# sasg/cilium

Hardware: AMD Instinct MI355X
Metric: classified headers/sec (Mpps, whole node) at 100k-prefix ipcache + 16k-ID policy (higher is better)
Workload: dtype u32

## Files before the change

### cilium_amd/csrc/classify.hip

```cpp
#include <algorithm>
#include <cstdlib>
#include <mutex>
#include <set>
#include <tuple>
#include <vector>

#include "kern_common.hpp"
#ifndef CFC_EXP
#define CFC_EXP 0
#endif

namespace cfc {

namespace {

constexpr int LDS_MET_U64 = 18;
template <int MODE>
constexpr int met_n()
{
    return MODE == CFC_MODE_EGRESS ? 7 : MODE == CFC_MODE_XDP ? 0 : 4;
}
template <int MODE>
constexpr int acc_n()
{
// ... 684 lines not shown
                          out.notify, o4);
                if (CT) {
                    sto_nt(h[u].ct_k1, C.ct, o4);
                    if (EGR)
                        sto_nt(h[u].ct_k2, C.ct2, o4);
                }
                if (LB && out.pkt_saddr) {
                    sto_nt(h[u].psa, out.pkt_saddr, o4);
                    sto_nt(h[u].da, out.pkt_daddr, o4);
                    sto_nt(h[u].ppt, out.pkt_ports, o4);
                }
                if (MODE != CFC_MODE_XDP) {
#if CFC_EXP != 3
                    if (!kc_ctr) {
                        sto_nt(ctr_key(C, h[u].ctr0, len), C.ctr, o4);
                        if (EGR)
                            sto_nt(ctr_key(C, h[u].ctr1, len), C.ctr2, o4);
                    }
                    if (!KC)
                        sto_nt(h[u].idw, C.id, o4);
#endif
                }
            }
#if CFC_EXP != 3
            if (MODE != CFC_MODE_XDP) {
                if (kc_ctr) {
                    key_append(ctr_key(C, h[u].ctr0, len), h[u].valid, C.ctr, kn_ctr);
                    if (EGR)
                        key_append(ctr_key(C, h[u].ctr1, len), h[u].valid, C.ctr2, kn_ctr2);
                }
                if (KC)
                    key_append(h[u].idw, h[u].valid, C.id, kn_id);
            }
#endif
            if (WL && E.wbits) {
                bool pr;
                const bool w = wl_want<EGR>(h[u].ct_byte, h[u].ver, h[u].mt, h[u].ct_k1,
                                            EGR ? h[u].ct_k2 : NONE, pr);
                const uint64_t wb = __ballot(w && h[u].valid), pb = __ballot(pr && h[u].valid);
                const uint32_t w0 = base + u * BLOCK + (threadIdx.x & ~63u);
                if ((threadIdx.x & 63) == 0 && w0 < end) {
                    E.wbits[(start + w0) >> 6] = wb;
                    E.wprobe[(start + w0) >> 6] = pb;
                }
            }
            if (MODE != CFC_MODE_XDP && E.nat_idx)
                list_append(E.nat_idx, E.nat_cnt, h[u].nat && h[u].valid, (uint32_t)start + i);
            if (MODE != CFC_MODE_XDP && h[u].valid && h[u].id_ovf && h[u].need_pol)
                id_count(C, id_dir, h[u].ident, h[u].drop1, len);
            if (LBE && h[u].valid && h[u].ver == DROP_NO_SERVICE) {
                unsigned long long *m = reinterpret_cast<unsigned long long *>(
                    C.g_met + (uint64_t)(-DROP_NO_SERVICE * METRIC_DIRS + METRIC_EGRESS) * 2);
                atomicAdd(m, 1ull);
                atomicAdd(m + 1, (unsigned long long)len);
            }
#if CFC_EXP != 5
            acc.add(h[u].valid ? h[u].met0 : NONE, len);
#endif
            if (EGR) {
                acc.add(h[u].valid ? h[u].met1 : NONE, len);
                acc.add(h[u].valid && h[u].ev2 ? met_n<MODE>() + h[u].ev2 - 1 : NONE, len);
            }
        }
        if (++iter == 65536 / (2 * U)) {
            acc.flush(s_met);
            iter = 0;
        }
    }
    acc.flush(s_met);
    if (CFC_KEYS_COMPACT && MODE != CFC_MODE_XDP && (threadIdx.x & 63) == 0) {
        const uint32_t wave = key_wave();
        const uint64_t to_counts =
            (uint64_t)(gridDim.x - blockIdx.x) * per_block -
            (uint64_t)wave * key_regions_grid(gridDim.x, per_block).cap +
            (uint64_t)blockIdx.x * KEY_WAVES + wave;
        if (kc_ctr) {
            C.ctr[to_counts] = kn_ctr;
            if (EGR)
                C.ctr2[to_counts] = kn_ctr2;
        }
        if (KC)
            C.id[to_counts] = kn_id;
    }
    __syncthreads();
    acc_publish<MODE>(s_met, C, E.seclabel);
}

}

namespace {

struct HistJob {
    const uint32_t *keys;
    uint64_t poff;
    uint32_t lo, cnt;
    uint32_t kind;
    uint32_t packed;
    uint32_t compact, cap;
    const uint32_t *counts;
    uint64_t n, per_block;
};
constexpr int HIST_JOBS_MAX = 12;
struct HistJobs {
    HistJob j[HIST_JOBS_MAX];
};
constexpr uint64_t SLICE_MAX = 1ull << 31;

__device__ __forceinline__ unsigned long long *hist_dst(const HistJob &jb, uint32_t key,
                                                        uint64_t *g_ctr, uint64_t *g_id,
                                                        uint32_t id_dir)
{
    return reinterpret_cast<unsigned long long *>(
        jb.kind == 0 ? g_ctr + 2ull * key : g_id + id_index(id_dir, key >> 1, key & 1));
}

struct HistLds {
    uint32_t *ek, *ec, *ew;
    uint32_t *s;
};
__device__ __forceinline__ HistLds hist_lds()
{
    uint32_t *b = reinterpret_cast<uint32_t *>(cfc_smem);
    return HistLds{b, b + HIST_ESC_SLOTS, b + 2 * HIST_ESC_SLOTS, b + 3 * HIST_ESC_SLOTS};
}

struct HistAdd {
    uint32_t r, len, old;
};
__device__ __forceinline__ HistAdd hist_add(uint32_t *s, const HistJob &jb, uint32_t w,
                                            uint32_t m)
{
    HistAdd a;
    uint32_t k;
    if (jb.packed) {
        k = w & 0xFFFF;
        a.len = w >> 16;
    } else {
        k = w;
        a.len = m >> 16;
    }
    a.r = k - jb.lo;
    a.old = a.r < jb.cnt && w != KEY_NONE ? atomicAdd(&s[a.r], HistSlot::inc(a.len)) : 0u;
    return a;
}
__device__ __forceinline__ bool hist_spills(const HistAdd &a)
{
    uint32_t carry, wrap;
    HistSlot::spill(a.old, a.len, carry, wrap);
    return (carry | wrap) != 0;
}
__device__ __forceinline__ void hist_escape(const HistLds &L, const HistJob &jb,
                                            const HistAdd &a, uint64_t *g_ctr, uint64_t *g_id,
                                            uint32_t id_dir)
{
    uint32_t carry, wrap;
    HistSlot::spill(a.old, a.len, carry, wrap);
    if (!(carry | wrap))
        return;
    uint32_t h = fmix32(a.r) & (HIST_ESC_SLOTS - 1);
    for (int p = 0; p < 8; p++) {
        uint32_t cur = L.ek[h];
        if (cur == NONE) {
            cur = atomicCAS(&L.ek[h], NONE, a.r);
            if (cur == NONE)
                cur = a.r;
        }
        if (cur == a.r) {
            if (carry)
                atomicAdd(&L.ec[h], carry);
            if (wrap)
                atomicAdd(&L.ew[h], wrap);
            return;
        }
        h = (h + 1) & (HIST_ESC_SLOTS - 1);
    }
    unsigned long long *d = hist_dst(jb, jb.lo + a.r, g_ctr, g_id, id_dir);
    atomicAdd(d, (unsigned long long)HistSlot::esc_packets(carry, wrap));
    if (carry)
        atomicAdd(d + 1, (unsigned long long)HistSlot::esc_bytes(carry));
}

__device__ __forceinline__ void hist_compact(const HistLds &L, const HistJob &jb,
                                             uint64_t start, uint64_t stop, uint64_t *g_ctr,
                                             uint64_t *g_id, uint32_t id_dir)
{
    if (start >= stop)
        return;
    const uint32_t wave = __builtin_amdgcn_readfirstlane(threadIdx.x >> 6);
    const uint32_t lane4 = 4 * (threadIdx.x & 63);
    const uint32_t r1 = (uint32_t)((stop + jb.cap - 1) / jb.cap);
    uint32_t r = (uint32_t)(start / jb.cap) + wave;
    uint32_t cnt = r < r1 ? jb.counts[r] : 0u;
    while (r < r1) {
        const uint32_t rn = r + KEY_WAVES;
        const uint32_t cnt_n = rn < r1 ? jb.counts[rn] : 0u;
        const uint64_t rb = (uint64_t)r * jb.cap;
        const uint64_t lo = max(rb, start), hi = min(rb + min(cnt, jb.cap), stop);
        if (lo < hi) {
            const uint32_t len = (uint32_t)(hi - lo), last = (len - 1) & ~3u;
            const uint32_t *k = jb.keys + lo;
            uint4 w0 = ld_nt4(k + min(lane4, last));
            uint4 w1 = ld_nt4(k + min(lane4 + 256, last));
            for (uint32_t o = lane4, b = 0; b < len; b += 256, o += 256) {
                const uint4 w2 = ld_nt4(k + min(o + 512, last));
                const HistAdd a0 = hist_add(L.s, jb, o < len ? w0.x : KEY_NONE, 0u);
                const HistAdd a1 = hist_add(L.s, jb, o + 1 < len ? w0.y : KEY_NONE, 0u);
                const HistAdd a2 = hist_add(L.s, jb, o + 2 < len ? w0.z : KEY_NONE, 0u);
                const HistAdd a3 = hist_add(L.s, jb, o + 3 < len ? w0.w : KEY_NONE, 0u);
                if (hist_spills(a0) | hist_spills(a1) | hist_spills(a2) | hist_spills(a3)) {
                    hist_escape(L, jb, a0, g_ctr, g_id, id_dir);
                    hist_escape(L, jb, a1, g_ctr, g_id, id_dir);
                    hist_escape(L, jb, a2, g_ctr, g_id, id_dir);
                    hist_escape(L, jb, a3, g_ctr, g_id, id_dir);
                }
                w0 = w1;
                w1 = w2;
            }
        }
        r = rn;
        cnt = cnt_n;
    }
}

__global__ __launch_bounds__(BLOCK) void k_hist(HistJobs J, const uint32_t *meta,
                                                uint32_t *partial, uint64_t *g_ctr,
                                                uint64_t *g_id, uint32_t id_dir)
{
    const HistJob jb = J.j[blockIdx.y];
    const HistLds L = hist_lds();
    uint32_t *s = L.s;
    for (uint32_t j = threadIdx.x; j < HIST_ESC_SLOTS; j += BLOCK) {
        L.ek[j] = NONE;
        L.ec[j] = 0;
        L.ew[j] = 0;
    }
    for (uint32_t j = threadIdx.x; j < jb.cnt; j += BLOCK)
        s[j] = 0;
    __syncthreads();
    const uint64_t start = (uint64_t)blockIdx.x * jb.per_block;
    const uint64_t stop = max(start, min(jb.n, start + jb.per_block));
    if (jb.compact)
        hist_compact(L, jb, start, stop, g_ctr, g_id, id_dir);
    const uint64_t end = jb.compact ? start : stop;
    const uint64_t end4 = start + ((end - start) & ~3ull);
    const bool meta16 = (reinterpret_cast<uintptr_t>(meta) & 15) == 0;
    auto load = [&](uint64_t i, uint4 &w, uint4 &m) {
        w = make_uint4(KEY_NONE, KEY_NONE, KEY_NONE, KEY_NONE);
        m = make_uint4(0, 0, 0, 0);
        if (i >= end4)
            return;
        w = ld_nt4(jb.keys + i);
        if (!jb.packed) {
            if (meta16) {
                m = ld_nt4(meta + i);
            } else {
                m.x = meta[i];
                m.y = meta[i + 1];
                m.z = meta[i + 2];
                m.w = meta[i + 3];
            }
        }
    };
    const uint64_t i0 = start + 4 * threadIdx.x;
    uint4 w0, m0, w1, m1;
    load(i0, w0, m0);
    load(i0 + 4 * BLOCK, w1, m1);
    for (uint64_t i = i0; i < end4; i += 4 * BLOCK) {
        uint4 w2, m2;
        load(i + 8 * BLOCK, w2, m2);
        const HistAdd a0 = hist_add(s, jb, w0.x, m0.x);
        const HistAdd a1 = hist_add(s, jb, w0.y, m0.y);
        const HistAdd a2 = hist_add(s, jb, w0.z, m0.z);
        const HistAdd a3 = hist_add(s, jb, w0.w, m0.w);
        if (hist_spills(a0) | hist_spills(a1) | hist_spills(a2) | hist_spills(a3)) {
            hist_escape(L, jb, a0, g_ctr, g_id, id_dir);
            hist_escape(L, jb, a1, g_ctr, g_id, id_dir);
            hist_escape(L, jb, a2, g_ctr, g_id, id_dir);
            hist_escape(L, jb, a3, g_ctr, g_id, id_dir);
        }
        w0 = w1; m0 = m1;
        w1 = w2; m1 = m2;
    }
    for (uint64_t i = end4 + threadIdx.x; i < end; i += BLOCK) {
        const HistAdd a = hist_add(s, jb, jb.keys[i], jb.packed ? 0u : meta[i]);
        if (hist_spills(a))
            hist_escape(L, jb, a, g_ctr, g_id, id_dir);
    }
    __syncthreads();
    uint32_t *dst = partial + jb.poff + (uint64_t)blockIdx.x * jb.cnt;
    for (uint32_t j = threadIdx.x; j < jb.cnt; j += BLOCK)
        st_nt(s[j], dst + j);
    for (uint32_t j = threadIdx.x; j < HIST_ESC_SLOTS; j += BLOCK) {
        const uint32_t r = L.ek[j];
        if (r == NONE)
            continue;
        const uint32_t carries = L.ec[j], wraps = L.ew[j];
        unsigned long long *d = hist_dst(jb, jb.lo + r, g_ctr, g_id, id_dir);
        atomicAdd(d, (unsigned long long)HistSlot::esc_packets(carries, wraps));
        if (carries)
            atomicAdd(d + 1, (unsigned long long)HistSlot::esc_bytes(carries));
    }
}

constexpr uint32_t REDUCE_ROWS = 32;
__global__ __launch_bounds__(256) void k_hist_reduce(HistJobs J, const uint32_t *partial,
                                                     uint32_t nblk, uint64_t *g_ctr,
                                                     uint64_t *g_id, uint32_t id_dir)
{
    const HistJob jb = J.j[blockIdx.y];
    const uint32_t j = blockIdx.x * 256 + threadIdx.x;
    if (j >= jb.cnt)
        return;
    uint64_t pk = 0, by = 0;
    const uint32_t *p = partial + jb.poff + j;
    const uint32_t b0 = blockIdx.z * REDUCE_ROWS, b1 = min(nblk, b0 + REDUCE_ROWS);
    for (uint32_t b = b0; b < b1; b++) {
        const uint32_t v = ld_nt(p + (uint64_t)b * jb.cnt);
        pk += HistSlot::packets(v);
        by += HistSlot::bytes(v);
    }
    if (!(pk | by))
        return;
    unsigned long long *dst = hist_dst(jb, jb.lo + j, g_ctr, g_id, id_dir);
    if (pk)
        atomicAdd(dst, (unsigned long long)pk);
    if (by)
        atomicAdd(dst + 1, (unsigned long long)by);
}

constexpr uint32_t CT_LDS_SLOTS = 8192;
constexpr uint32_t CT_LDS_BYTES = CT_LDS_SLOTS * 12;
__global__ __launch_bounds__(BLOCK) void k_ct_count(const uint32_t *ct_idx,
                                                    const uint32_t *ct_idx2,
                                                    const uint32_t *meta,
                                                    uint64_t n,
                                                    CtState *st)
{
    uint32_t *keys = reinterpret_cast<uint32_t *>(cfc_smem);
    unsigned long long *vals =
        reinterpret_cast<unsigned long long *>(keys + CT_LDS_SLOTS);
    for (uint32_t j = threadIdx.x; j < CT_LDS_SLOTS; j += BLOCK) {
        keys[j] = NONE;
        vals[j] = 0;
    }
    __syncthreads();
    const uint32_t *idx = blockIdx.y ? ct_idx2 : ct_idx;
    const uint64_t start = (uint64_t)blockIdx.x * COUNT_PER_BLOCK;
    const uint64_t end = min(n, start + COUNT_PER_BLOCK);
    for (uint64_t i = start + threadIdx.x; i < end; i += BLOCK) {
        const uint32_t k = ld_nt(idx + i);
        if (k >= CK_MISS)
            continue;
        const uint32_t len = ld_nt(meta + i) >> 16;
        uint32_t h = fmix32(k) & (CT_LDS_SLOTS - 1);
        bool done = false;
        for (int p = 0; p < 8 && !done; p++) {
            uint32_t cur = keys[h];
            if (cur == NONE) {
                cur = atomicCAS(&keys[h], NONE, k);
                if (cur == NONE)
                    cur = k;
            }
            if (cur == k) {
                atomicAdd(&vals[h], (1ull << 32) | len);
                done = true;
            }
            h = (h + 1) & (CT_LDS_SLOTS - 1);
        }
        if (!done) {
            unsigned long long *a = ct_acct_at(st, k);
            atomicAdd(a, 1ull);
            atomicAdd(a + 1, (unsigned long long)len);
        }
    }
    __syncthreads();
    for (uint32_t j = threadIdx.x; j < CT_LDS_SLOTS; j += BLOCK) {
        const uint32_t k = keys[j];
        const unsigned long long v = vals[j];
        if (k != NONE && v) {
            unsigned long long *a = ct_acct_at(st, k);
            atomicAdd(a, v >> 32);
            atomicAdd(a + 1, v & 0xFFFFFFFFull);
        }
    }
}

constexpr uint32_t CTP_BUCKET_BITS = 12, CTP_BUCKET = 1u << CTP_BUCKET_BITS;
constexpr uint32_t CTP_MAX_BUCKETS = 32768;
constexpr uint32_t ACC_FINE_BITS = 7, ACC_FINE = 1u << ACC_FINE_BITS;
constexpr uint32_t ACC_MAX_COARSE = CTP_MAX_BUCKETS / ACC_FINE;
constexpr int ACC_KEY_SHIFT = 37, ACC_KIND_BIT = 36, ACC_BY_BITS = 20;
constexpr uint32_t ACC_BY_MASK = (1u << ACC_BY_BITS) - 1;
constexpr uint32_t ACC_CHUNK_BITS = 14, ACC_CHUNK = 1u << ACC_CHUNK_BITS;
constexpr uint32_t ACC_PER_THREAD = ACC_CHUNK / BLOCK;
constexpr uint32_t ACC_SLICE_CHUNKS = 5;
constexpr uint32_t ACC_RCAP = ACC_SLICE_CHUNKS * ACC_CHUNK;
static_assert(COUNT_PER_BLOCK + 2 * CT_LDS_SLOTS <= ACC_RCAP, "slice records");
static_assert(CTP_BUCKET % BLOCK == 0, "reduce flush");
constexpr int ACC_COARSE_SHIFT = ACC_KEY_SHIFT + CTP_BUCKET_BITS + ACC_FINE_BITS;
constexpr int ACC_BUCKET_SHIFT = ACC_KEY_SHIFT + CTP_BUCKET_BITS;
static_assert(ACC_COARSE_SHIFT + 8 == 64, "coarse bucket: the key's top 8 bits");
constexpr uint32_t ACC_AGG_LDS =
    CT_LDS_SLOTS * 16 + ACC_SLICE_CHUNKS * ACC_MAX_COARSE * 4 + 16;
constexpr uint32_t ACC_SORT_LDS = ACC_CHUNK * 8 + 3 * ACC_MAX_COARSE * 4 + 16;
constexpr uint32_t ACC_RED_LDS = CTP_BUCKET * 16;

uint64_t acc_slice(uint64_t n)
{
    const uint64_t full = 256ull * COUNT_PER_BLOCK;
    if (n <= full)
        return COUNT_PER_BLOCK;
    const uint64_t rounds = (n + full - 1) / full;
    const uint64_t per = (n + 256 * rounds - 1) / (256 * rounds);
    return (per + 3) & ~3ull;
}

__device__ __forceinline__ uint64_t acc_rec(uint32_t k, uint32_t pk, uint32_t by)
{
    return (uint64_t)k << ACC_KEY_SHIFT | (uint64_t)pk << ACC_BY_BITS | by;
}
__device__ __forceinline__ uint64_t acc_rec1(uint32_t k, bool one, uint32_t fl, uint32_t low)
{
    return (uint64_t)k << ACC_KEY_SHIFT | 1ull << ACC_KIND_BIT | (one ? 1ull << 25 : 0ull) |
           (uint64_t)fl << 16 | low;
}
__device__ __forceinline__ uint32_t acc_flags(uint32_t meta, uint32_t tf)
{
    const bool tcp = (meta & 0xFF) == 6;
    return tcp ? ((tf & 0xFF) | ((meta & CFC_HF_TCP_CLOSE) ? 0u : 0x100u)) : 0u;
}

__device__ __forceinline__ uint32_t wave_append(uint32_t *ctr, bool want)
{
    const uint64_t m = __ballot(want);
    const uint32_t lane = threadIdx.x & 63;
    const uint32_t lead = m ? (uint32_t)__builtin_ctzll(m) : 0u;
    uint32_t base = 0;
    if (m && lane == lead)
        base = atomicAdd(ctr, (uint32_t)__popcll(m));
    base = __shfl(base, (int)lead, 64);
    return base + (uint32_t)__popcll(m & ((1ull << lane) - 1));
}
constexpr int CTP_PROBES = 3;

template <bool VEC>
__global__ __launch_bounds__(BLOCK) void k_acc_agg(const uint32_t *ct_idx,
                                                   const uint32_t *ct_idx2,
                                                   const uint32_t *meta, const uint8_t *tf,
                                                   bool sums, uint64_t n,
                                                   uint32_t nco, uint64_t *rec,
                                                   uint32_t *rcnt, uint32_t *cnt, uint64_t per)
{
    uint32_t *keys = reinterpret_cast<uint32_t *>(cfc_smem);
    unsigned long long *vals = reinterpret_cast<unsigned long long *>(keys + CT_LDS_SLOTS);
    uint32_t *fls = reinterpret_cast<uint32_t *>(vals + CT_LDS_SLOTS);
    uint32_t *hist = fls + CT_LDS_SLOTS;
    uint32_t *nrec = hist + ACC_SLICE_CHUNKS * ACC_MAX_COARSE;
    for (uint32_t j = threadIdx.x; j < CT_LDS_SLOTS; j += BLOCK) {
        keys[j] = NONE;
        vals[j] = 0;
        fls[j] = 0;
    }
    for (uint32_t j = threadIdx.x; j < ACC_SLICE_CHUNKS * ACC_MAX_COARSE; j += BLOCK)
        hist[j] = 0;
    if (threadIdx.x == 0)
        *nrec = 0;
    __syncthreads();
    const uint32_t nv = gridDim.x * gridDim.y;
    const uint32_t vw = blockIdx.y * gridDim.x + blockIdx.x;
    const uint32_t *idx = blockIdx.y ? ct_idx2 : ct_idx;
    uint64_t *rs = rec + (uint64_t)vw * ACC_RCAP;
    const uint64_t start = (uint64_t)blockIdx.x * per;
    const uint64_t end = min(n, start + per);
    auto put = [&](uint32_t r, uint64_t v) {
        rs[r] = v;
        atomicAdd(&hist[(r >> ACC_CHUNK_BITS) * ACC_MAX_COARSE + (uint32_t)(v >> ACC_COARSE_SHIFT)],
                  1u);
    };
    auto one = [&](uint32_t k, uint32_t len, uint32_t fl) {
        uint32_t h = fmix32(k) & (CT_LDS_SLOTS - 1);
        bool done = k >= CK_MISS;
        for (int p = 0; p < CTP_PROBES && !done; p++) {
            uint32_t cur = keys[h];
            if (cur == NONE) {
                cur = atomicCAS(&keys[h], NONE, k);
                if (cur == NONE)
                    cur = k;
            }
            if (cur == k) {
                atomicAdd(&vals[h], (1ull << 32) | len);
                if (fl && (fls[h] & fl) != fl)
                    atomicOr(&fls[h], fl);
                done = true;
            }
            h = (h + 1) & (CT_LDS_SLOTS - 1);
        }
        const uint32_t r = wave_append(nrec, !done);
        if (!done)
            put(r, acc_rec1(k, true, fl, len));
    };
    constexpr uint32_t W = VEC ? 4 : 1, STEP = W * BLOCK;
    auto load = [&](uint64_t e, uint4 &kk, uint4 &mm, uint32_t &ff) {
        if (VEC && e + 4 <= end) {
            kk = ld_nt4(idx + e);
            mm = ld_nt4(meta + e);
            ff = tf ? ld_nt(reinterpret_cast<const uint32_t *>(tf + e)) : 0u;
        } else {
            kk = make_uint4(NONE, NONE, NONE, NONE);
            mm = make_uint4(0, 0, 0, 0);
            ff = 0;
            if (e < end) { kk.x = ld_nt(idx + e); mm.x = ld_nt(meta + e); ff = tf ? tf[e] : 0u; }
            if (VEC && e + 1 < end) {
                kk.y = ld_nt(idx + e + 1); mm.y = ld_nt(meta + e + 1);
                ff |= tf ? (uint32_t)tf[e + 1] << 8 : 0u;
            }
            if (VEC && e + 2 < end) {
                kk.z = ld_nt(idx + e + 2); mm.z = ld_nt(meta + e + 2);
                ff |= tf ? (uint32_t)tf[e + 2] << 16 : 0u;
            }
        }
    };
    const uint64_t e0 = start + (uint64_t)threadIdx.x * W;
    uint4 k0, m0, k1, m1;
    uint32_t f0, f1;
    load(e0, k0, m0, f0);
    load(e0 + STEP, k1, m1, f1);
    for (uint64_t i0 = start; i0 < end; i0 += STEP) {
        uint4 k2, m2;
        uint32_t f2;
        load(e0 + (i0 - start) + 2 * STEP, k2, m2, f2);
        one(k0.x, m0.x >> 16, sums ? acc_flags(m0.x, f0) : 0u);
        if (VEC) {
            one(k0.y, m0.y >> 16, sums ? acc_flags(m0.y, f0 >> 8) : 0u);
            one(k0.z, m0.z >> 16, sums ? acc_flags(m0.z, f0 >> 16) : 0u);
            one(k0.w, m0.w >> 16, sums ? acc_flags(m0.w, f0 >> 24) : 0u);
        }
        k0 = k1; m0 = m1; f0 = f1;
        k1 = k2; m1 = m2; f1 = f2;
    }
    __syncthreads();
    for (uint32_t j = threadIdx.x; j < CT_LDS_SLOTS; j += BLOCK) {
        const uint32_t k = keys[j];
        const unsigned long long v = vals[j];
        const uint32_t by = (uint32_t)v, fl = fls[j];
        const uint32_t r = wave_append(nrec, k != NONE);
        if (k != NONE)
            put(r, acc_rec(k, (uint32_t)(v >> 32), by & ACC_BY_MASK));
        const bool hi = k != NONE && (by > ACC_BY_MASK || fl);
        const uint32_t r2 = wave_append(nrec, hi);
        if (hi)
            put(r2, acc_rec1(k, false, fl, by >> ACC_BY_BITS));
    }
    __syncthreads();
    const uint32_t nch = nv * ACC_SLICE_CHUNKS;
    for (uint32_t j = threadIdx.x; j < nco * ACC_SLICE_CHUNKS; j += BLOCK) {
        const uint32_t c = j / ACC_SLICE_CHUNKS, q = j % ACC_SLICE_CHUNKS;
        cnt[(uint64_t)c * nch + vw * ACC_SLICE_CHUNKS + q] = hist[q * ACC_MAX_COARSE + c];
    }
    if (threadIdx.x == 0)
        rcnt[vw] = *nrec;
}

__device__ __forceinline__ void acc_local_sort(const uint64_t (&r)[ACC_PER_THREAD], uint32_t m,
                                               int shift, uint32_t mask, uint32_t nd,
                                               uint64_t *buf, uint32_t *cnt, uint32_t *base)
{
    for (uint32_t j = threadIdx.x; j < nd; j += BLOCK)
        cnt[j] = 0;
    __syncthreads();
    uint32_t rank[ACC_PER_THREAD];
#pragma unroll
    for (uint32_t i = 0; i < ACC_PER_THREAD; i++) {
        const uint32_t x = threadIdx.x + i * BLOCK;
        if (x < m)
            rank[i] = atomicAdd(&cnt[(uint32_t)(r[i] >> shift) & mask], 1u);
    }
    __syncthreads();
    static_assert(ACC_MAX_COARSE <= 256, "one wave scans four counts per lane");
    if (threadIdx.x < 64) {
        const uint32_t l = threadIdx.x;
        uint32_t v[4], x = 0;
#pragma unroll
        for (int q = 0; q < 4; q++) {
            v[q] = 4 * l + q < nd ? cnt[4 * l + q] : 0u;
            x += v[q];
        }
        const uint32_t own = x;
#pragma unroll
        for (int d = 1; d < 64; d <<= 1) {
            const uint32_t y = __shfl_up(x, d, 64);
            if (l >= (uint32_t)d)
                x += y;
        }
        uint32_t e = x - own;
#pragma unroll
        for (int q = 0; q < 4; q++) {
            if (4 * l + q < nd)
                base[4 * l + q] = e;
            e += v[q];
        }
        if (l == 63)
            base[nd] = x;
    }
    __syncthreads();
#pragma unroll
    for (uint32_t i = 0; i < ACC_PER_THREAD; i++) {
        const uint32_t x = threadIdx.x + i * BLOCK;
        if (x < m)
            buf[base[(uint32_t)(r[i] >> shift) & mask] + rank[i]] = r[i];
    }
    __syncthreads();
}

__global__ __launch_bounds__(BLOCK) void k_acc_part1(const uint64_t *rec, const uint32_t *rcnt,
                                                     const uint32_t *off, uint32_t nch,
                                                     uint32_t nco, uint64_t *outA)
{
    uint64_t *buf = reinterpret_cast<uint64_t *>(cfc_smem);
    uint32_t *cnt = reinterpret_cast<uint32_t *>(buf + ACC_CHUNK);
    uint32_t *base = cnt + ACC_MAX_COARSE;
    uint32_t *goff = base + ACC_MAX_COARSE + 1;
    const uint32_t ch = blockIdx.x, vw = ch / ACC_SLICE_CHUNKS, q = ch % ACC_SLICE_CHUNKS;
    const uint32_t all = rcnt[vw], lo = q * ACC_CHUNK;
    if (lo >= all)
        return;
    const uint32_t m = min(ACC_CHUNK, all - lo);
    const uint64_t *src = rec + (uint64_t)vw * ACC_RCAP + lo;
    for (uint32_t c = threadIdx.x; c < nco; c += BLOCK)
        goff[c] = off[(uint64_t)c * nch + ch];
    uint64_t r[ACC_PER_THREAD];
// ... 345 lines not shown
}

uint64_t hist_slots(const DevTables &T, int mode)
{
    if (mode == CFC_MODE_XDP)
        return 0;
    uint64_t id_slots = 0;
    for (uint32_t r = 0; r < ID_RANGES; r++)
        if ((T.id_cover >> r) & 1)
            id_slots += std::min<uint64_t>(2 * ID_RANGE, 2ull * ID_PACK_LIMIT - 2ull * r * ID_RANGE);
    return (mode == CFC_MODE_EGRESS ? 2ull : 1ull) * T.n_ctr + id_slots;
}

}

void set_lds_limit(const void *kernel, int bytes)
{
    static std::mutex mu;
    static std::set<std::tuple<int, const void *, int>> done;
    int dev = 0;
    (void)hipGetDevice(&dev);
    std::lock_guard<std::mutex> g(mu);
    if (done.insert(std::make_tuple(dev, kernel, bytes)).second)
        (void)hipFuncSetAttribute(kernel, hipFuncAttributeMaxDynamicSharedMemorySize,
                                  bytes);
}

size_t classify_lds_bytes(const DevTables &T) { return lds_plan(T).bytes(); }

int launch_patch16(const Patch16 *rec, uint64_t n, hipStream_t s)
{
    if (!n)
        return 0;
    hipLaunchKernelGGL(k_patch16, dim3((unsigned)((n + 255) / 256)), dim3(256), 0, s, rec, n);
    return hipGetLastError() == hipSuccess ? 0 : -5;
}

int launch_add_u64(uint64_t *dst, const uint64_t *src, uint64_t n,
                   hipStream_t s)
{
    if (!n)
        return 0;
    hipLaunchKernelGGL(k_add_u64, dim3((unsigned)((n + 255) / 256)), dim3(256),
                       0, s, dst, src, n);
    return hipGetLastError() == hipSuccess ? 0 : -5;
}

uint32_t ctp_buckets(const DevTables &T)
{
    if (getenv("CFC_ACC_PER_SLICE"))
        return 0;
    const uint64_t slots = (T.ct4 ? T.ct4_mask + 1ull : 0) + (T.ct6 ? T.ct6_mask + 1ull : 0);
    const uint64_t nb = (2 * slots + CTP_BUCKET - 1) / CTP_BUCKET;
    return nb <= CTP_MAX_BUCKETS ? (uint32_t)nb : 0u;
}

WsLayout ws_layout(uint64_t n, const DevTables &T, int mode, bool ct, int num_cus)
{
    WsLayout w{};
    if (n == 0 || mode == CFC_MODE_XDP)
        return w;
    const bool egr = mode == CFC_MODE_EGRESS;
    const size_t a = 4 * ctr_stride(n);
    w.key_pb = key_per_block(n, (uint64_t)std::max(num_cus, 1) * CFC_WG_PER_CU,
                             (uint64_t)BLOCK * CFC_UNROLL);
    const size_t ka = std::max<size_t>(a, 4 * key_regions(n, w.key_pb).words());
    size_t off = 0;
    w.ctr = off;
    off += ka;
    if (egr) {
        w.ctr2 = off;
        off += ka;
    }
    w.id = off;
    off += ka;
    if (ct) {
        w.ct = off;
        off += a;
        if (egr) {
            w.ct2 = off;
            off += a;
        }
    }
    off = (off + 255) & ~(size_t)255;
    w.partial = off;
    const uint64_t slots = hist_slots(T, mode);
    w.nblk = hist_slices(n, slots);
    off += 4ull * slots * w.nblk;
    const uint32_t nbuck = ctp_buckets(T);
    if (ct && T.ct_st && nbuck) {
        const uint64_t per = acc_slice(n);
        const uint32_t nblk = (uint32_t)((n + per - 1) / per);
        w.ctp_nv = nblk * (egr ? 2u : 1u);
        w.ctp_nbuck = nbuck;
        w.ctp_nco = (nbuck + ACC_FINE - 1) / ACC_FINE;
        const uint64_t cap = (uint64_t)w.ctp_nv * ACC_RCAP;
        const uint64_t nc = (uint64_t)w.ctp_nco * w.ctp_nv * ACC_SLICE_CHUNKS;
        w.ctp_g2 = (uint32_t)((cap + ACC_CHUNK - 1) / ACC_CHUNK + w.ctp_nco);
        auto take = [&](size_t bytes) {
            off = (off + 255) & ~(size_t)255;
            const size_t at = off;
            off += bytes;
            return at;
        };
        w.ctp_rec = take(8 * cap);
        w.ctp_recA = take(8 * cap);
        w.ctp_rcnt = take(4ull * w.ctp_nv);
        w.ctp_cnt = take(4 * nc);
        w.ctp_off = take(4 * nc + 4);
        w.ctp_bsum = take(4 * ((nc + 4 * BLOCK - 1) / (4 * BLOCK)) + 4);
        w.ctp_plan = take(4ull * (2 * w.ctp_nco + 2));
        w.ctp_fo = take(4ull * w.ctp_g2 * (ACC_FINE + 1));
    }
    if (egr && (T.lb4 || T.rnat4)) {
        off = (off + 255) & ~(size_t)255;
        w.lb = off;
        off += 6 * a;
    }
    w.total = off;
    return w;
}

CountArgs count_args(uint32_t *ws, const WsLayout &w, const DevTables &T,
                     uint64_t *g_met, int mode, bool ct, bool v4)
{
    CountArgs C{};
    char *b = reinterpret_cast<char *>(ws);
    if (w.total) {
        C.ctr = reinterpret_cast<uint32_t *>(b + w.ctr);
        C.ctr2 = mode == CFC_MODE_EGRESS ? reinterpret_cast<uint32_t *>(b + w.ctr2) : nullptr;
        C.id = reinterpret_cast<uint32_t *>(b + w.id);
        C.ct = ct ? reinterpret_cast<uint32_t *>(b + w.ct) : nullptr;
        C.ct2 = ct && mode == CFC_MODE_EGRESS ? reinterpret_cast<uint32_t *>(b + w.ct2)
                                              : nullptr;
    }
    C.g_met = g_met;
    C.g_id = g_met + METRIC_U64;
    C.ctr_packed = T.n_ctr < PACK_MAX;
    if (v4 && w.total)
        C.compact = CFC_KEYS_COMPACT & (KEYS_ID | (C.ctr_packed ? KEYS_CTR : 0u));
    return C;
}

int launch_classify_v4(const DevTables &T, const cfc_hdr_v4 &in,
                       const cfc_out &out, int mode, const EgressArgs &E,
                       uint64_t *g_ctr, uint32_t *ws, int num_cus, hipStream_t s,
                       const LaunchTiming *tm, const uint32_t *tr_id)
{
    if (in.n == 0)
        return 0;
    if (classify_lds_bytes(T) > LDS_PER_WG)
        return -22;
    const uint64_t per_block = key_per_block(in.n, (uint64_t)std::max(num_cus, 1) * CFC_WG_PER_CU,
                                             (uint64_t)BLOCK * CFC_UNROLL);
    const uint32_t grid = (uint32_t)((in.n + per_block - 1) / per_block);
    if (tm)
        (void)hipEventRecord(tm->ev[0], s);
    const bool lb = (T.lb4 || T.rnat4) && mode != CFC_MODE_XDP;
    const bool ct = T.ct4 || out.ct || lb;
    const WsLayout w = ws_layout(in.n, T, mode, ct, num_cus);
    const CountArgs C = count_args(ws, w, T, g_ctr + 2ull * T.n_ctr, mode, ct, true);
    cfc_hdr_v4 hin = in;
    LbIn li{};
    if (lb && mode == CFC_MODE_EGRESS) {
        uint32_t *a = reinterpret_cast<uint32_t *>(reinterpret_cast<char *>(ws) + w.lb);
        const uint64_t st = ctr_stride(in.n);
        LbArgs A{in.saddr, in.daddr, in.ports, in.meta, in.hash, in.n, E.lxc_id,
                 E.ct_owner, a, a + st, a + 2 * st, a + 3 * st, a + 4 * st, a + 5 * st, E.svo};
        if (int rc = launch_lb4_egress(T, A, s))
            return rc;
        li = LbIn{A.tda, A.tpt, A.psa, A.fl};
        hin.daddr = A.pda;
        hin.ports = A.ppt;
    } else if (out.pkt_saddr && !lb) {
        if (hipMemcpyAsync(out.pkt_saddr, in.saddr, 4 * in.n, hipMemcpyDeviceToDevice, s) ||
            hipMemcpyAsync(out.pkt_daddr, in.daddr, 4 * in.n, hipMemcpyDeviceToDevice, s) ||
            hipMemcpyAsync(out.pkt_ports, in.ports, 4 * in.n, hipMemcpyDeviceToDevice, s))
            return -5;
    }
    const LbIn *lbp = lb ? &li : nullptr;
#define CFC_LAUNCH(M)                                                        \
    (ct ? launch_mode<M, true>(T, hin, out, E, C, grid, per_block, s, lbp, tr_id)   \
        : launch_mode<M, false>(T, hin, out, E, C, grid, per_block, s, lbp, tr_id))
    switch (mode) {
    case CFC_MODE_INGRESS: CFC_LAUNCH(CFC_MODE_INGRESS); break;
    case CFC_MODE_EGRESS: CFC_LAUNCH(CFC_MODE_EGRESS); break;
    case CFC_MODE_XDP:
        launch_mode<CFC_MODE_XDP, false>(T, hin, out, E, C, grid, per_block, s, nullptr, nullptr);
        break;
    case CFC_MODE_FULL: CFC_LAUNCH(CFC_MODE_FULL); break;
    default: return -22;
    }
#undef CFC_LAUNCH
    if (tm)
        (void)hipEventRecord(tm->ev[1], s);
    const bool sums = launch_counters(T, in.meta, in.tcp_flags, in.n, mode, ws, g_ctr, s, ct,
                                      C, w);
    if (E.sums)
        *E.sums = sums;
    if (tm)
        (void)hipEventRecord(tm->ev[2], s);
    hipError_t e = hipGetLastError();
    return e == hipSuccess ? 0 : -5;
}

bool launch_counters(const DevTables &T, const uint32_t *meta, const uint8_t *tf, uint64_t n,
                     int mode, uint32_t *ws, uint64_t *g_ctr, hipStream_t s,
                     bool ct, const CountArgs &C, const WsLayout &w)
{
    bool sums = false;
    if (!n || mode == CFC_MODE_XDP)
        return sums;
    if (ct && T.ct_st && w.ctp_nv) {
        char *b = reinterpret_cast<char *>(ws);
        uint64_t *rec = reinterpret_cast<uint64_t *>(b + w.ctp_rec);
        uint64_t *recA = reinterpret_cast<uint64_t *>(b + w.ctp_recA);
        uint32_t *rcnt = reinterpret_cast<uint32_t *>(b + w.ctp_rcnt);
        uint32_t *cnt = reinterpret_cast<uint32_t *>(b + w.ctp_cnt);
        uint32_t *off = reinterpret_cast<uint32_t *>(b + w.ctp_off);
        uint32_t *bsum = reinterpret_cast<uint32_t *>(b + w.ctp_bsum);
        uint32_t *plan = reinterpret_cast<uint32_t *>(b + w.ctp_plan);
        uint32_t *fo = reinterpret_cast<uint32_t *>(b + w.ctp_fo);
        const uint64_t per = acc_slice(n);
        const uint32_t nblk = (uint32_t)((n + per - 1) / per);
        const uint32_t nch = w.ctp_nv * ACC_SLICE_CHUNKS;
        const uint64_t nc = (uint64_t)w.ctp_nco * nch;
        const uint32_t nsb = (uint32_t)((nc + 4 * BLOCK - 1) / (4 * BLOCK));
        const bool vec = ((uintptr_t)meta & 15) == 0 && (!T.ct_sum || ((uintptr_t)tf & 3) == 0);
        const void *agg = vec ? (const void *)k_acc_agg<true> : (const void *)k_acc_agg<false>;
        set_lds_limit(agg, (int)ACC_AGG_LDS);
        if (vec)
            hipLaunchKernelGGL(k_acc_agg<true>, dim3(nblk, mode == CFC_MODE_EGRESS ? 2 : 1),
                               dim3(BLOCK), ACC_AGG_LDS, s, C.ct, C.ct2, meta,
                               T.ct_sum ? tf : nullptr, T.ct_sum != nullptr, n,
                               w.ctp_nco, rec, rcnt, cnt, per);
        else
            hipLaunchKernelGGL(k_acc_agg<false>, dim3(nblk, mode == CFC_MODE_EGRESS ? 2 : 1),
                               dim3(BLOCK), ACC_AGG_LDS, s, C.ct, C.ct2, meta,
                               T.ct_sum ? tf : nullptr, T.ct_sum != nullptr, n,
                               w.ctp_nco, rec, rcnt, cnt, per);
        hipLaunchKernelGGL(k_scan_local, dim3(nsb), dim3(BLOCK), 0, s, cnt, off, nc, bsum);
        hipLaunchKernelGGL(k_scan_top, dim3(1), dim3(BLOCK), 0, s, bsum, nsb, off + nc);
        hipLaunchKernelGGL(k_scan_add, dim3(nsb), dim3(BLOCK), 0, s, off, nc, bsum);
        set_lds_limit((const void *)k_acc_part1, (int)ACC_SORT_LDS);
        hipLaunchKernelGGL(k_acc_part1, dim3(nch), dim3(BLOCK), ACC_SORT_LDS, s, rec, rcnt,
                           off, nch, w.ctp_nco, recA);
        hipLaunchKernelGGL(k_acc_plan, dim3(1), dim3(64), 0, s, off, nch, w.ctp_nco, plan);
        set_lds_limit((const void *)k_acc_part2, (int)ACC_SORT_LDS);
        hipLaunchKernelGGL(k_acc_part2, dim3(w.ctp_g2), dim3(BLOCK), ACC_SORT_LDS, s, recA,
                           plan, w.ctp_nco, rec, fo);
        set_lds_limit((const void *)k_acc_reduce, (int)ACC_RED_LDS);
        hipLaunchKernelGGL(k_acc_reduce, dim3(w.ctp_nbuck), dim3(BLOCK), ACC_RED_LDS, s, rec,
                           plan, fo, w.ctp_nco, T.ct_st, T.ct_sum);
        sums = T.ct_sum != nullptr;
    } else if (ct && T.ct_st) {
        set_lds_limit((const void *)k_ct_count, (int)CT_LDS_BYTES);
        const uint32_t nblk = (uint32_t)((n + COUNT_PER_BLOCK - 1) / COUNT_PER_BLOCK);
        hipLaunchKernelGGL(k_ct_count, dim3(nblk, mode == CFC_MODE_EGRESS ? 2 : 1),
                           dim3(BLOCK), CT_LDS_BYTES, s, C.ct, C.ct2, meta, n, T.ct_st);
    }
    std::vector<HistJob> jobs;
    uint64_t poff = 0;
    const KeyRegions KG = key_regions(n, w.key_pb);
    auto job = [&](const uint32_t *keys, uint32_t lo, uint32_t cnt, uint32_t kind,
                   uint32_t packed, bool compact) {
        HistJob j{};
        j.keys = keys;
        j.poff = poff;
        j.lo = lo;
        j.cnt = cnt;
        j.kind = kind;
        j.packed = packed;
        j.compact = compact;
        j.cap = compact ? KG.cap : 0u;
        j.counts = compact ? keys + KG.counts() : nullptr;
        j.n = compact ? KG.extent : n;
        j.per_block = hist_per_block(j.n, w.nblk);
        poff += (uint64_t)w.nblk * j.cnt;
        jobs.push_back(j);
    };
    auto add_jobs = [&](const uint32_t *keys, uint32_t nkeys) {
        for (uint32_t lo = 0; lo < nkeys; lo += HIST_RANGE)
            job(keys, lo, std::min(HIST_RANGE, nkeys - lo), 0, C.ctr_packed,
                (C.compact & KEYS_CTR) != 0);
    };
    add_jobs(C.ctr, T.n_ctr);
    if (mode == CFC_MODE_EGRESS)
        add_jobs(C.ctr2, T.n_ctr);
    for (uint32_t r = 0; r < ID_RANGES; r++) {
        if (!((T.id_cover >> r) & 1))
            continue;
        const uint32_t lo = 2 * r * ID_RANGE;
        job(C.id, lo, std::min(2 * ID_RANGE, 2 * ID_PACK_LIMIT - lo), 1, 1,
            (C.compact & KEYS_ID) != 0);
    }
    if (jobs.empty())
        return sums;
    uint32_t *partial = reinterpret_cast<uint32_t *>(reinterpret_cast<char *>(ws) + w.partial);
    set_lds_limit((const void *)k_hist, (int)(HIST_ESC_BYTES + 4 * HIST_RANGE));
    const uint32_t id_dir = mode == CFC_MODE_EGRESS ? ID_DIR_EGRESS : ID_DIR_INGRESS;
    for (size_t a = 0; a < jobs.size(); a += HIST_JOBS_MAX) {
        HistJobs J{};
        const uint32_t nj = (uint32_t)std::min<size_t>(HIST_JOBS_MAX, jobs.size() - a);
        uint32_t cmax = 0;
        for (uint32_t k = 0; k < nj; k++) {
            J.j[k] = jobs[a + k];
            cmax = std::max(cmax, J.j[k].cnt);
        }
        hipLaunchKernelGGL(k_hist, dim3(w.nblk, nj), dim3(BLOCK),
                           HIST_ESC_BYTES + 4ull * cmax, s, J, meta, partial, g_ctr, C.g_id,
                           id_dir);
        hipLaunchKernelGGL(k_hist_reduce,
                           dim3((cmax + 255) / 256, nj, (w.nblk + REDUCE_ROWS - 1) / REDUCE_ROWS),
                           dim3(256), 0, s, J, partial, w.nblk, g_ctr, C.g_id, id_dir);
    }
    return sums;
}

}
```

Before: 62570.

## Restructure histogram reduce with vector loads, wave-split rows and LDS combine

Rewrites the partial-histogram reduction kernel so each lane handles four adjacent slots through 128-bit non-temporal loads when offsets are aligned. The four waves of a block split the row range, with an unroll of eight for memory-level parallelism, and their sums are combined in shared memory before the global atomics. Rows per z-slice grow from 32 to 256, which cuts the atomic traffic per slot. The cost is fewer blocks in flight and accumulation in u32, which is bounded by a static assert.

```diff
diff --git a/cilium_amd/csrc/classify.hip b/cilium_amd/csrc/classify.hip
--- a/cilium_amd/csrc/classify.hip
+++ b/cilium_amd/csrc/classify.hip
@@ -1010,30 +1010,101 @@
     }
 }
 
-constexpr uint32_t REDUCE_ROWS = 32;
-__global__ __launch_bounds__(256) void k_hist_reduce(HistJobs J, const uint32_t *partial,
-                                                     uint32_t nblk, uint64_t *g_ctr,
-                                                     uint64_t *g_id, uint32_t id_dir)
+#ifndef CFC_REDUCE_ROWS
+#define CFC_REDUCE_ROWS 256
+#endif
+constexpr uint32_t REDUCE_ROWS = CFC_REDUCE_ROWS;
+constexpr uint32_t REDUCE_UNROLL = 8;
+constexpr uint32_t REDUCE_WAVES = 4;
+static_assert(REDUCE_ROWS <= 2048, "k_hist_reduce sums a group's fields in u32");
+__host__ __device__ inline bool hist_reduce_vec(uint64_t poff, uint32_t cnt)
+{
+    return ((poff | cnt) & 3) == 0;
+}
+__host__ __device__ inline uint32_t hist_reduce_keys(uint64_t poff, uint32_t cnt)
+{
+    return 64u * (hist_reduce_vec(poff, cnt) ? 4u : 1u);
+}
+
+template <uint32_t K>
+__device__ __forceinline__ void hist_reduce_job(const HistJob &jb, const uint32_t *partial,
+                                                uint32_t nblk, uint64_t *g_ctr, uint64_t *g_id,
+                                                uint32_t id_dir)
+{
+    __shared__ uint32_t s_pk[REDUCE_WAVES][64 * K], s_by[REDUCE_WAVES][64 * K];
+    const uint32_t k0 = blockIdx.x * 64 * K;
+    if (k0 >= jb.cnt)
+        return;
+    const uint32_t wave = threadIdx.x >> 6, lane = threadIdx.x & 63;
+    const uint32_t j = k0 + K * lane;
+    const uint32_t b0 = blockIdx.z * REDUCE_ROWS, b1 = min(nblk, b0 + REDUCE_ROWS);
+    uint32_t pk[K], by[K];
+#pragma unroll
+    for (uint32_t k = 0; k < K; k++)
+        pk[k] = by[k] = 0;
+    if (j < jb.cnt) {
+        const uint32_t *p = partial + jb.poff + j;
+        for (uint32_t b = b0 + wave; b < b1; b += REDUCE_WAVES * REDUCE_UNROLL) {
+            uint32_t v[REDUCE_UNROLL][K];
+#pragma unroll
+            for (uint32_t u = 0; u < REDUCE_UNROLL; u++) {
+                const uint32_t row = b + REDUCE_WAVES * u;
+#pragma unroll
+                for (uint32_t k = 0; k < K; k++)
+                    v[u][k] = 0;
+                if (row < b1) {
+                    if constexpr (K == 4) {
+                        const uint4 q = ld_nt4(p + (uint64_t)row * jb.cnt);
+                        v[u][0] = q.x; v[u][1] = q.y; v[u][2] = q.z; v[u][3] = q.w;
+                    } else {
+                        v[u][0] = ld_nt(p + (uint64_t)row * jb.cnt);
+                    }
+                }
+            }
+#pragma unroll
+            for (uint32_t u = 0; u < REDUCE_UNROLL; u++)
+#pragma unroll
+                for (uint32_t k = 0; k < K; k++) {
+                    pk[k] += (uint32_t)HistSlot::packets(v[u][k]);
+                    by[k] += (uint32_t)HistSlot::bytes(v[u][k]);
+                }
+        }
+    }
+#pragma unroll
+    for (uint32_t k = 0; k < K; k++) {
+        s_pk[wave][K * lane + k] = pk[k];
+        s_by[wave][K * lane + k] = by[k];
+    }
+    __syncthreads();
+    for (uint32_t t = threadIdx.x; t < 64 * K; t += 64 * REDUCE_WAVES) {
+        if (k0 + t >= jb.cnt)
+            break;
+        uint64_t spk = 0, sby = 0;
+#pragma unroll
+        for (uint32_t w = 0; w < REDUCE_WAVES; w++) {
+            spk += s_pk[w][t];
+            sby += s_by[w][t];
+        }
+        if (!(spk | sby))
+            continue;
+        unsigned long long *dst = hist_dst(jb, jb.lo + k0 + t, g_ctr, g_id, id_dir);
+        if (spk)
+            atomicAdd(dst, (unsigned long long)spk);
+        if (sby)
+            atomicAdd(dst + 1, (unsigned long long)sby);
+    }
+}
+
+__global__ __launch_bounds__(64 * REDUCE_WAVES) void k_hist_reduce(HistJobs J,
+                                                                   const uint32_t *partial,
+                                                                   uint32_t nblk, uint64_t *g_ctr,
+                                                                   uint64_t *g_id, uint32_t id_dir)
 {
     const HistJob jb = J.j[blockIdx.y];
-    const uint32_t j = blockIdx.x * 256 + threadIdx.x;
-    if (j >= jb.cnt)
-        return;
-    uint64_t pk = 0, by = 0;
-    const uint32_t *p = partial + jb.poff + j;
-    const uint32_t b0 = blockIdx.z * REDUCE_ROWS, b1 = min(nblk, b0 + REDUCE_ROWS);
-    for (uint32_t b = b0; b < b1; b++) {
-        const uint32_t v = ld_nt(p + (uint64_t)b * jb.cnt);
-        pk += HistSlot::packets(v);
-        by += HistSlot::bytes(v);
-    }
-    if (!(pk | by))
-        return;
-    unsigned long long *dst = hist_dst(jb, jb.lo + j, g_ctr, g_id, id_dir);
-    if (pk)
-        atomicAdd(dst, (unsigned long long)pk);
-    if (by)
-        atomicAdd(dst + 1, (unsigned long long)by);
+    if (hist_reduce_vec(jb.poff, jb.cnt))
+        hist_reduce_job<4>(jb, partial, nblk, g_ctr, g_id, id_dir);
+    else
+        hist_reduce_job<1>(jb, partial, nblk, g_ctr, g_id, id_dir);
 }
 
 constexpr uint32_t CT_LDS_SLOTS = 8192;
@@ -1985,17 +2056,19 @@
     for (size_t a = 0; a < jobs.size(); a += HIST_JOBS_MAX) {
         HistJobs J{};
         const uint32_t nj = (uint32_t)std::min<size_t>(HIST_JOBS_MAX, jobs.size() - a);
-        uint32_t cmax = 0;
+        uint32_t cmax = 0, rgrid = 0;
         for (uint32_t k = 0; k < nj; k++) {
             J.j[k] = jobs[a + k];
             cmax = std::max(cmax, J.j[k].cnt);
+            const uint32_t per = hist_reduce_keys(J.j[k].poff, J.j[k].cnt);
+            rgrid = std::max(rgrid, (J.j[k].cnt + per - 1) / per);
         }
         hipLaunchKernelGGL(k_hist, dim3(w.nblk, nj), dim3(BLOCK),
                            HIST_ESC_BYTES + 4ull * cmax, s, J, meta, partial, g_ctr, C.g_id,
                            id_dir);
         hipLaunchKernelGGL(k_hist_reduce,
-                           dim3((cmax + 255) / 256, nj, (w.nblk + REDUCE_ROWS - 1) / REDUCE_ROWS),
-                           dim3(256), 0, s, J, partial, w.nblk, g_ctr, C.g_id, id_dir);
+                           dim3(rgrid, nj, (w.nblk + REDUCE_ROWS - 1) / REDUCE_ROWS),
+                           dim3(64 * REDUCE_WAVES), 0, s, J, partial, w.nblk, g_ctr, C.g_id, id_dir);
     }
     return sums;
 }
```

Result: faster. 63210, median of 6 (+1.0%).
